# DTUWindEnergy/WindGym

Measured on AMD Instinct MI355X. Metric: env-steps/sec (whole node), 16-turbine farm x 4096 envs, higher is better.
Workload: dtype f32

## Files before the change

windgym_amd/csrc/wg_env.hip:

```cpp
#include <hip/hip_runtime.h>

#ifndef WG_ENV_ABLATE
#define WG_ENV_ABLATE 0
#endif
#include "wg_env_common.h"
#include "wg_internal.h"

struct __attribute__((aligned(16))) EnvSlotLds {
    int dev_rem, fill_rem, sub, budget;
    double s_new;
    int n_emit, n_valid, new_valid;
    unsigned n_emitted;
    float s_off_f, near_f, move_max, ti_pow;
    double s_off, ws;
    float ws_f, ti_f, wd_env, base_acc;
    int n_pushed, pend_farm_n, pend_base_n, n_flow;
    double c_time;
    int c_head;
    unsigned c_part, c_flow, c_istep, c_tag, n_emitted0;
    float out_pw;
    unsigned c_add;
    int bg_init;
    int pad_[3];
};
static_assert(sizeof(EnvSlotLds) == WG_ENV_SLOT_LDS_BYTES, "keep WG_ENV_SLOT_LDS_BYTES in sync (wg_flow.h)");
#define WG_ENV_OFF_SRC4 0
#define WG_ENV_OFF_REC4 1024
#define WG_ENV_OFF_RING 2048
#define WG_ENV_OFF_XR 3072
#define WG_ENV_OFF_SRC2 3584
#define WG_ENV_OFF_SL 4096
#define WG_ENV_OFF_HDR (WG_ENV_OFF_SL + 4 * WG_ENV_SLOT_LDS_BYTES)
#define WG_ENV_OFF_STAGE (WG_ENV_OFF_HDR + 128)
static_assert(WG_ENV_OFF_STAGE == WG_ENV_FIXED_LDS_BYTES, "keep WG_ENV_FIXED_LDS_BYTES in sync (wg_flow.h)");

__device__ __forceinline__ float env_slot_sums(const float v, const int N, const int NS, const int k, const int tid) {
    if (N == 16) return wg_row_sum(v);
    if (N < 16) {
        const int r = tid >> 4, i = tid & 15;
        const float x = __shfl(v, (r * N + i) & 63, 64);
        const float s = wg_row_sum((i < N && r < NS) ? x : 0.f);
        return __shfl(s, k << 4, 64);
    }
    const int h = tid >> 5, i = tid & 31;
    const float x = __shfl(v, (h * N + i) & 63, 64);
    float s = (i < N && h < NS) ? x : 0.f;
    WG_ROW_REDUCE(s, wg_addf)
    s += __shfl_xor(s, 16, 64);
    return __shfl(s, k << 5, 64);
}

static __device__ __forceinline__ void env_clone_dev(char* const smem, const int kd, const int N, const int P, const double dt_d,
                                                               float* const py_env, unsigned* const ra_env, const unsigned src,
                                                               const unsigned dst, const int lane) {
    float4* const Lsrc4 = reinterpret_cast<float4*>(smem + WG_ENV_OFF_SRC4);
    int4* const Lring = reinterpret_cast<int4*>(smem + WG_ENV_OFF_RING);
    float2* const Lsrc2 = reinterpret_cast<float2*>(smem + WG_ENV_OFF_SRC2);
    EnvSlotLds* const SL = reinterpret_cast<EnvSlotLds*>(smem + WG_ENV_OFF_SL);
    const int ga = (kd - 1) * N, gb = kd * N;
    const int4 last = Lring[ga + N - 1];
    const int nq = (last.x + last.y) >> 2;
    {
        const float4* const ps = reinterpret_cast<const float4*>(py_env + src);
        float4* const pd = reinterpret_cast<float4*>(py_env + dst);
        const uint4* const rs = reinterpret_cast<const uint4*>(ra_env + 2 * (size_t)src);
        uint4* const rd = reinterpret_cast<uint4*>(ra_env + 2 * (size_t)dst);
#pragma unroll 2
        for (int q = lane; q < nq; q += 64) {
            const float4 y = ps[q];
            const uint4 r0 = rs[q], r1 = rs[q + nq];
            pd[q] = y; rd[q] = r0; rd[q + nq] = r1;
        }
    }
    if (lane < N) {
        Lsrc4[gb + lane] = Lsrc4[ga + lane];
        Lsrc2[gb + lane] = Lsrc2[ga + lane];
        Lring[gb + lane].z = Lring[ga + lane].z;
    }
    if (lane == 0) {
        const EnvSlotLds& a = SL[kd - 1];
        EnvSlotLds& b = SL[kd];
        b.n_valid = a.n_valid; b.n_emitted = a.n_emitted; b.s_off = a.s_off;
        b.dev_rem = 0; b.sub = 0;
        b.budget = a.budget;
        double tm = a.c_time;
        for (int i = 0; i < a.n_flow; ++i) tm += dt_d;
        b.c_time = tm;
        int hd = a.c_head + (int)((a.n_emitted - a.n_emitted0) % (unsigned)P); if (hd >= P) hd -= P;
        b.c_head = hd; b.n_emitted0 = a.n_emitted;
        b.c_istep = a.c_istep + (unsigned)a.n_flow;
    }
}

template <bool NOISE, int WPE, int GLUE, int SPLIT>
__device__ __forceinline__ void env_flow(char* const smem, char* const smem_pass, float* const zone, const int wv, const int role, const int mode,
                                         const float* __restrict__ actions, const uint8_t* __restrict__ mask, const int chunk, EnvFlowOut& out) {
    const int tid = threadIdx.x & 63, e = blockIdx.x;
    int N, F, NS, NL;
    float inv_N;
    {
        const KArgsPtr ka = wg_cold_args();
        N = ka->p.N; F = ka->p.F; inv_N = ka->p.inv_N;
        NS = WPE == 2 ? F : 2 * F; NL = NS * N;
    }
    const int kbase = WPE == 2 ? wv * F : 0;
    const bool valid = tid < NL;
    const int g = valid ? tid : 0;
    const int k = (int)(((float)g + 0.5f) * inv_N);
    const int t = g - k * N;
    const int c = WPE == 2 ? wv : (F == 2 ? (k >> 1) : k), farm = F == 2 ? (k & 1) : 0;

    float4* const Lsrc4 = reinterpret_cast<float4*>(smem + WG_ENV_OFF_SRC4);
    uint4* const Lrec4 = reinterpret_cast<uint4*>(smem + WG_ENV_OFF_REC4);
    int4* const Lring = reinterpret_cast<int4*>(smem + WG_ENV_OFF_RING);
    double* const Lxr = reinterpret_cast<double*>(smem + WG_ENV_OFF_XR);
    float2* const Lsrc2 = reinterpret_cast<float2*>(smem + WG_ENV_OFF_SRC2);
    EnvSlotLds* const SL = reinterpret_cast<EnvSlotLds*>(smem + WG_ENV_OFF_SL);
    float* const def = reinterpret_cast<float*>(smem + WG_ENV_OFF_STAGE);
    float* const tiav = def + WG_ENV_CAP;
    unsigned short* const cl = reinterpret_cast<unsigned short*>(tiav + WG_ENV_CAP);
    unsigned short* const ql = reinterpret_cast<unsigned short*>(smem + WG_ENV_OFF_STAGE);
    EnvSlotLds& my = SL[k];

    WG_STAMP(0);
// ... 111 lines not shown
                const int dev0 = __shfl(dev_rem, WPE == 2 ? 0 : (env_live ^ 1) * F * N, 64);
                budget = wg_shadow_share(dev0 + gp.K * fill_max, total - env_steps_done, env_steps_done, e);
                budget = wg_shadow_share(dev_rem + gp.K * fill_rem, total - env_steps_done, env_steps_done, e, farm ? 0x80000000u : 0u);
                plan_left = total - env_steps_done;
            } else {
                const int inc = k0->p.env_inc;
                const long total = (long)((env_time_max_live + inc - 1) / inc) + 1;
                budget = role_dev ? wg_shadow_share(dev_rem + k0->p.K * fill_rem, total - env_steps_done, env_steps_done, e, farm ? 0x80000000u : 0u) : 0;
                plan_left = total - env_steps_done;
            }
        } else {
            role_dev = is_live_c && !masked_out;
            budget = chunk;
        }
        bool clone_here = false;
        if (k0->p.env_share) {
            const int dev_a = __shfl(dev_rem, (tid - N) & 63, 64);
            parked = valid && role_dev && farm == 1 && dev_rem > 0 && c_istep == 0u && dev_a > 0;
            const int twin_fill = __shfl(parked ? fill_rem + 1 : 0, (tid + N) & 63, 64);
            const bool lead = valid && role_dev && farm == 0 && twin_fill > 0;
            if (lead && mode == WG_MODE_STEP && !defer_init)
                budget = wg_shadow_share(dev_rem + k0->p.K * max(fill_rem, twin_fill - 1), plan_left, env_steps_done, e);
            if (parked) budget = 0;
            clone_here = lead && budget >= dev_rem;
        }
        if (SPLIT) {
            const bool two = valid && role_dev && budget >= 2;
            split_on = mode == WG_MODE_STEP && k0->p.K == 1 && (is_live_c || (SPLIT == 2 && !out.bg_init_pending)) && !defer_init && !__ballot(two) &&
                       !__ballot(clone_here);
            if (role == 1 && !split_on) return;
        }
        if (WPE == 2 && valid && t == 0) {
            my.dev_rem = dev_rem; my.fill_rem = fill_rem; my.bg_init = out.bg_init_pending; my.n_flow = 0; my.out_pw = 0.f;
        }
        {
            const bool any_work = valid && (role_live || (role_dev && budget > 0 && (dev_rem > 0 || fill_rem > 0)));
            if (!__ballot(any_work)) {
                if (WPE == 2 && mode == WG_MODE_STEP && !is_live_c && autoreset && role == 0) {
                    const int d0 = __shfl(dev_rem, 0, 64), f0 = __shfl(fill_rem, 0, 64), np0 = __shfl(n_pushed, 0, 64);
                    const KArgsPtr kf = wg_cold_args();
                    if (d0 == 0 && f0 == 0 && kf->d.gd->next_obs_ok != nullptr && kf->d.gd->next_obs_ok[ctx_id] == 0) {
                        out.first_obs = 1;
                        env_first_obs<GLUE != 0>((int)ctx_id, np0, tid);
                    }
                }
                return;
            }
        }

        const KArgsPtr k1 = wg_cold_args();
        const int rlen = l_rnext - l_roff;
        const int head = n_emitted == 0u ? rlen - 1 : fast_mod((int)(n_emitted - 1u), rlen, __builtin_amdgcn_rcpf((float)rlen));
        const float ws_f = (float)ws;
        if (valid) {
            Lxr[g] = l_xr;
            Lsrc4[g] = make_float4((float)l_xr, (float)l_yr, l_bnd.y, l_bnd.z);
            Lsrc2[g] = make_float2(l_bnd.x, l_bnd.w);
            Lring[g] = make_int4(l_roff, rlen, head, k);
            Lrec4[g] = make_uint4(0u, 0u, 0u, __float_as_uint(1.f));
            if (t == 0) {
                my.dev_rem = dev_rem; my.fill_rem = fill_rem; my.sub = 0; my.budget = budget;
                my.n_valid = n_valid; my.n_emitted = n_emitted; my.n_emitted0 = n_emitted;
                my.move_max = fabsf(k1->p.hill) * ws_f * k1->p.dt; my.ti_pow = fast_pow(ti_f, k1->p.tic);
                my.s_off = s_off; my.ws = ws; my.ws_f = ws_f; my.ti_f = ti_f; my.wd_env = wd_env; my.base_acc = 0.f;
                my.n_pushed = n_pushed; my.pend_farm_n = pend_farm_n; my.pend_base_n = pend_base_n; my.n_flow = 0;
                my.bg_init = out.bg_init_pending;
                my.c_time = c_time; my.c_head = c_head; my.c_part = c_part; my.c_flow = c_flow; my.c_istep = c_istep; my.c_tag = c_tag; my.c_add = c_add;
            }
        }
        float* const tabp = reinterpret_cast<float*>(smem + k1->p.env_off_tab);
        float* const tabct = tabp + n_tab;
        float2* const rpt = reinterpret_cast<float2*>(tabct + n_tab);
        const float hub = k1->p.hub;
        auto rp = [&](const float dy_, const float dz_) __attribute__((always_inline)) {
            const float dz = hub + dz_ - hub;
            return make_float2(dy_, dz * dz);
        };
        if (tid < n_tab) { tabp[tid] = pf_tp; tabct[tid] = pf_tc; }
        if (tid < S) rpt[tid] = rp(pf_dy, pf_dz);
        for (int i = tid + 64; i < n_tab; i += 64) { tabp[i] = k1->d.tab_power[i]; tabct[i] = k1->d.tab_ct[i]; }
        for (int i = tid + 64; i < S; i += 64) rpt[i] = rp(k1->d.rotor_dy[i], k1->d.rotor_dz[i]);

        yaw = l_yaw; tu = l_u; tti = l_ti; oyaw = l_yaw;
        if (role_live && farm == 0 && valid) {
            const float a = l_act, ymin = k1->p.yaw_min, ymax = k1->p.yaw_max, ystep = k1->p.yaw_step;
            if (k1->p.action_method == WG_ACT_YAW) {
                yaw = fminf(fmaxf(yaw + a * ystep, ymin), ymax);
            } else {
                float tf = a + 1.0f;
                tf = tf * 0.5f;
                tf = tf * (ymax - ymin);
                tf = tf + ymin;
                const float ny = fminf(fmaxf(tf, yaw - ystep), yaw + ystep);
                yaw = fminf(fmaxf(ny, ymin), ymax);
            }
        }
    }
    float tpow = 0.f, tct = 0.f, cg = 1.f;
    float sws = 0.f, swd = 0.f, syaw = 0.f, sp_ = 0.f;
    int part_acc = 0, stream_acc = 0;
    bool stepped = false;
    lds_barrier<64>();
    WG_STAMP(1);

    for (int round = 0;; ++round) {
        bool stepping, is_dev;
        int sub, K;
        if (__ballot(parked)) {
            bool due = parked && SL[k - 1].dev_rem == 0;
            unsigned long long due_m = __ballot(due);
            if (due_m) {
                full_barrier<64>();
                const KArgsPtr kc = wg_cold_args();
                const unsigned pstride = (unsigned)kc->p.pstride;
                const size_t pb_env = (size_t)(e * 2 * F + kbase) * pstride;
                const int src_lane = (tid - N) & 63;
                const float c_tu = __shfl(tu, src_lane, 64), c_tti = __shfl(tti, src_lane, 64), c_pw = __shfl(tpow, src_lane, 64);
                const float c_ct = __shfl(tct, src_lane, 64), c_cg = __shfl(cg, src_lane, 64);
                if (due) { tu = c_tu; tti = c_tti; tpow = c_pw; tct = c_ct; cg = c_cg; stepped = true; parked = false; }
                while (due_m) {
                    const int kd = __builtin_amdgcn_readlane(k, __builtin_ctzll(due_m));
                    env_clone_dev(smem, kd, N, kc->p.P, kc->p.dt_d, kc->d.py + pb_env, kc->d.rec_a + 2 * pb_env, (unsigned)(kd - 1) * pstride,
                                  (unsigned)kd * pstride, tid);
                    due_m &= ~(((1ull << N) - 1ull) << (kd * N));
                }
                lds_barrier<64>();
            }
        }
        {
            const KArgsPtr kr = wg_cold_args();
            K = kr->p.K;
            const int4 sch = *reinterpret_cast<const int4*>(&my.dev_rem);
            const bool active = sch.x > 0 || sch.y > 0;
            stepping = valid && (role_live ? (round < K) : (role_dev && active && (sch.w > 0 || sch.z != 0)));
            is_dev = !role_live && sch.x > 0;
            sub = sch.z;
            if (!__ballot(stepping)) break;
        out.rounds = round + 1;
            if (round > 0) full_barrier<64>();

            if (role_live && farm == 1 && stepping) {
                const float ystep = kr->p.yaw_step;
                if (kr->p.base_controller == WG_CTRL_LOCAL) {
                    const float off = 0.f - yaw;
                    const float sgn = (float)((off > 0.f) - (off < 0.f));
                    yaw = yaw + sgn * fminf(fabsf(off), ystep);
                } else {
                    const float sgn = (float)((yaw > 0.f) - (yaw < 0.f));
                    yaw = yaw - sgn * fminf(fabsf(yaw), ystep);
                }
            }

            if (stepping && t == 0) {
                const double dpart = kr->p.dpart;
                const int P = kr->p.P;
                const double s_off = my.s_off, adv = my.ws * kr->p.dt_d;
                double s_new = s_off + adv;
                int n_emit = 0;
                while (s_new >= dpart) { s_new -= dpart; ++n_emit; }
                if (n_emit > P) n_emit = P;
                int new_valid = my.n_valid + n_emit; if (new_valid > P) new_valid = P;
                my.s_new = s_new; my.n_emit = n_emit; my.new_valid = new_valid;
                my.s_off_f = (float)s_off;
                my.near_f = (float)(s_off + adv + dpart) + 0.01f;
            }
        }
        lds_barrier<64>();
        WG_STAMP(4);

        unsigned cmask = 0u;
        {
            const KArgsPtr kp = wg_cold_args();
            const float D = kp->p.D, inv_D = kp->p.inv_D, eps_max = kp->p.env_eps_max;
            const int gs0 = k * N;
            const float lim0 = kp->p.R_rot + 1.0e-3f * D;
            const float near_f = my.near_f, move_max = my.move_max;
            const float xt_f = Lsrc4[g].x, yt_f = Lsrc4[g].y;
#pragma unroll 4
            for (int s2 = 0; s2 < N; ++s2) {
                const float4 a = Lsrc4[gs0 + s2];
                const float2 b = Lsrc2[gs0 + s2];
                const float dxf = xt_f - a.x;
                const bool nearp = dxf < near_f;
                const float kb_ = nearp ? fmaxf(WG_K_MAX, a.z) : a.z, eb_ = nearp ? fmaxf(eps_max, a.w) : a.w;
                const float sig_max = (kb_ * (dxf * inv_D) + eb_) * D;
                const float bdv = b.x + (((__float_as_uint(b.y) != 0u) | nearp) ? move_max : 0.f);
                const float gap = fabsf(yt_f - a.y) - (5.0f * sig_max + bdv);
                const bool cd = (s2 != t) & (dxf >= 0.f) & (gap <= lim0);
                cmask |= cd ? (1u << s2) : 0u;
            }
            if (!stepping || (SPLIT && role == 1)) cmask = 0u;
        }
        int cbeg, nc;
        {
            const int cnt = __popc(cmask);
            const int inc = wg_wave_scan_i(cnt);
            cbeg = inc - cnt;
            nc = __builtin_amdgcn_readlane(inc, 63);
            unsigned m = cmask;
            int o = cbeg;
            while (m) { cl[o++] = (unsigned short)((g << 5) | __builtin_ctz(m)); m &= m - 1u; }
        }
        lds_barrier<64>();
        WG_STAMP(5);

        struct Cand { uint2 q0, q1; float y0, y1, xd, wgt; int en, jp0; bool ok, rest; };
        float dsum = 0.f, tia_max = 0.f;
        {
            const KArgsPtr kp = wg_cold_args();
            const unsigned pstride = (unsigned)kp->p.pstride;
            const size_t pb_env = (size_t)(e * 2 * F + kbase) * pstride;
            const uint2* const rc_env = reinterpret_cast<const uint2*>(kp->d.rec_a + 2 * pb_env);
            const float* const py_env = kp->d.py + pb_env;
            const double inv_dpart = kp->p.inv_dpart;
            const float inv_D = kp->p.inv_D;
            auto issue = [&](Cand& cd, const int cidx, const int c0, const int c1) __attribute__((always_inline)) {
                cd.ok = false; cd.rest = false;
// ... 155 lines not shown
            if (stepping) {
                const int4 rg = Lring[g];
                const unsigned mvl = __float_as_uint(Lsrc2[g].y);
                const int n_emit = my.n_emit;
                const bool full = (mvl != 0u && (int)(my.n_emitted - mvl) < rg.y) || n_emit >= 4 || n_emit >= rg.y;
                stream_acc += full ? rg.y : n_emit;
            }
        }
        if (stepping) {
            const float ti_f = my.ti_f;
            tu = my.ws_f;
            tu -= dsum;
            tti = __builtin_amdgcn_sqrtf(ti_f * ti_f + tia_max * tia_max);
        }
        lds_barrier<64>();
        WG_STAMP(9);

        if (!(SPLIT && split_on && role == 0)) {
            const KArgsPtr kp = wg_cold_args();
            const unsigned pstride = (unsigned)kp->p.pstride;
            const size_t pb_env = (size_t)(e * 2 * F + kbase) * pstride;
            float* const py_env = kp->d.py + pb_env;
            unsigned* const ra_env = kp->d.rec_a + 2 * pb_env;
            int nlist;
            {
                int cnt = 0, nqd = 0;
                bool full = false;
                if (stepping) {
                    const int4 rg = Lring[g];
                    const int rlen = rg.y, n_emit = my.n_emit;
                    const unsigned mvl = __float_as_uint(Lsrc2[g].y);
                    nqd = rlen >> 2;
                    const bool moving = mvl != 0u && (int)(my.n_emitted - mvl) < rlen;
                    full = moving || n_emit >= 4 || n_emit >= rlen;
                    stream_acc += full ? rlen : n_emit;
                    if (full) cnt = nqd;
                    else if (n_emit > 0) {
                        const unsigned sb = (unsigned)k * pstride + (unsigned)rg.x;
                        const uint4 rn = Lrec4[g];
                        const float y0 = Lsrc4[g].y;
#pragma unroll
                        for (int em = 0; em < 3; ++em) {
                            if (em < n_emit) {
                                int r = rg.z + 1 + em; if (r >= rlen) r -= rlen;
                                const unsigned ix = sb + (unsigned)r;
                                py_env[ix] = y0;
                                reinterpret_cast<uint2*>(ra_env)[ix] = make_uint2(rn.x, rn.y);
                            }
                        }
                    }
                }
                const int inc = wg_wave_scan_i(cnt);
                nlist = (WG_ENV_ABLATE & 2) ? 0 : __builtin_amdgcn_readlane(inc, 63);
                if (full) {
                    const int base = inc - cnt;
                    const unsigned tag = (unsigned)g << 10;
                    for (int i = 0; i < nqd; ++i) ql[base + i] = (unsigned short)(tag | (unsigned)i);
                }
            }
            lds_barrier<64>();
            WG_STAMP(10);
#ifdef WG_TIMELINE
            if (tid == 0) atomicAdd(&wg_counts[4], nlist);
#endif

            const float dpart_f = kp->p.dpart_f, inv_D = kp->p.inv_D, dt = kp->p.dt, eps0 = kp->p.eps0;
            struct QuadReq { float4 py; uint4 ra, rb; int g, kq; unsigned q; };
            auto request = [&](QuadReq& r, const int cidx) __attribute__((always_inline)) {
                const bool v = cidx < nlist;
                const unsigned en = v ? ql[cidx] : 0u;
                r.g = (int)(en >> 10); r.kq = (int)(en & 1023u);
                const int4 rg = Lring[r.g];
                r.q = (((unsigned)rg.w * pstride + (unsigned)rg.x) >> 2) + (unsigned)r.kq;
                if (v) {
                    r.py = reinterpret_cast<const float4*>(py_env)[r.q];
                    r.ra = reinterpret_cast<const uint4*>(ra_env)[2u * r.q];
                    r.rb = reinterpret_cast<const uint4*>(ra_env)[2u * r.q + 1u];
                }
            };
            auto advect_quad = [&](const QuadReq& cur, const int cidx) __attribute__((always_inline)) {
                if (cidx >= nlist) return;
                const int gq = cur.g, kq = cur.kq;
                const unsigned q = cur.q;
                const int4 rg = Lring[gq];
                const EnvSlotLds& sl = SL[rg.w];
                const int n_emit_q = sl.n_emit, n_valid_q = sl.n_valid;
                const float sof = sl.s_off_f;
                const int R = rg.y, hd = rg.z;
                const int r0 = 4 * kq;
                int j0 = hd - r0; if (j0 < 0) j0 += R;
                int e0 = r0 - hd - 1; if (e0 < 0) e0 += R;
                const bool emits = (e0 < n_emit_q) || (n_emit_q > 0 && e0 + 3 >= R);
                float pyv[4] = {cur.py.x, cur.py.y, cur.py.z, cur.py.w};
                unsigned rav[4] = {cur.ra.x, cur.ra.z, cur.rb.x, cur.rb.z};
                unsigned rbv[4] = {cur.ra.y, cur.ra.w, cur.rb.y, cur.rb.w};
#pragma unroll
                for (int i = 0; i < 4; ++i) {
                    int j = j0 - i; if (j < 0) j += R;
                    const float adv = m0_advect(pyv[i], rav[i], rbv[i], j, sof, dpart_f, inv_D, dt, eps0);
                    pyv[i] = j < n_valid_q ? adv : pyv[i];
                }
                const float y0 = Lsrc4[gq].y;
                if (emits) {
                    const uint4 rn = Lrec4[gq];
#pragma unroll
                    for (int i = 0; i < 4; ++i) {
                        int ei = e0 + i; if (ei >= R) ei -= R;
                        if (ei < n_emit_q) {
                            pyv[i] = y0; rav[i] = rn.x; rbv[i] = rn.y;
                        }
                    }
                    reinterpret_cast<uint4*>(ra_env)[2u * q] = make_uint4(rav[0], rbv[0], rav[1], rbv[1]);
                    reinterpret_cast<uint4*>(ra_env)[2u * q + 1u] = make_uint4(rav[2], rbv[2], rav[3], rbv[3]);
                }
                reinterpret_cast<float4*>(py_env)[q] = make_float4(pyv[0], pyv[1], pyv[2], pyv[3]);
                float ex = 0.f;
#pragma unroll
                for (int i = 0; i < 4; ++i) {
                    int j = j0 - i; if (j < 0) j += R;
                    if (j < n_valid_q) ex = fmaxf(ex, fabsf(pyv[i] - y0));
                }
                if (ex > Lsrc2[gq].x) atomicMax(reinterpret_cast<int*>(&Lsrc2[gq].x), __float_as_int(ex));
            };
            QuadReq qa, qb;
            qa.py = qb.py = make_float4(0.f, 0.f, 0.f, 0.f); qa.ra = qa.rb = qb.ra = qb.rb = make_uint4(0u, 0u, 0u, 0u);
            request(qa, tid);
            if (SPLIT && role == 1) {
                if (!env_flag_wait(reinterpret_cast<int*>(smem + WG_ENV_OFF_HDR))) atomicOr(kp->d.status, WG_STATUS_BIT_STATE);
            }
            for (int base = 0; base < nlist; base += 64) {
                qb = qa;
                request(qa, base + 64 + tid);
                advect_quad(qb, base + tid);
            }
        }
        lds_barrier<64>();
        WG_STAMP(3);
        if (SPLIT && role == 1) {
            if (stepping) reinterpret_cast<float4*>(wg_cold_args()->d.bnd)[(unsigned)((e * 2 * F + kbase) * N + g)].x = Lsrc2[g].x;
            return;
        }

        const bool measuring = stepping && !is_dev;
        const bool unit_end = measuring && (sub + 1 == K);
        const KArgsPtr kc = wg_cold_args();
        const float inv_k = 1.0f / (float)K;
        const unsigned ctx_id = (unsigned)(e * 2 + c);
        if (stepping) {
            {
                int4 rg = Lring[g];
                const int n_emit = my.n_emit;
                rg.z += n_emit;
                if (n_emit >= rg.y) rg.z %= rg.y; else if (rg.z >= rg.y) rg.z -= rg.y;
                Lring[g].z = rg.z;
                part_acc += min(my.new_valid, rg.y);
            }
            stepped = true;
            const int n_tab = kc->p.n_tab;
            const float tab_x0 = kc->p.tab_x0, tab_inv_dx = kc->p.tab_inv_dx;
            const float* const tabp = reinterpret_cast<const float*>(smem + kc->p.env_off_tab);
            const float wsn = fmaxf(tu * cg, 0.0f);
            tpow = env_tab(tabp, tab_x0, tab_inv_dx, n_tab, wsn);
            tct = env_tab(tabp + n_tab, tab_x0, tab_inv_dx, n_tab, wsn) * cg * cg;
            if (measuring && farm == 0) {
                const float wsm = __builtin_amdgcn_sqrtf(tu * tu);
                const float wdm = 0.f + my.wd_env;
                float val[WG_N_CH] = {sws + wsm, swd + wdm, syaw + yaw, sp_ + tpow};
                if (unit_end) {
// ... 101 lines not shown
            for (int i = 0; i < n_flow; ++i) tm += dt_d;
            const unsigned n_emitted = my.n_emitted;
            int hd = my.c_head + (int)((n_emitted - my.n_emitted0) % (unsigned)P); if (hd >= P) hd -= P;
            WgSlot& slot = ke->d.slot[(unsigned)(e * 2 * F + kbase + k)];
            slot.part_count = my.c_part + (unsigned)part_slot;
            slot.add_count = my.c_add + (unsigned)stream_slot;
            slot.head = hd; slot.n_valid = my.n_valid; slot.s_off = my.s_off; slot.time = tm;
            slot.istep = my.c_istep + (unsigned)n_flow; slot.n_emitted = n_emitted;
            slot.dev_remaining = my.dev_rem; slot.fill_remaining = my.fill_rem;
            slot.flow_count = my.c_flow + (unsigned)n_flow;
            WgCtx& cx = ke->d.ctx[(unsigned)(e * 2 + c)];
            if (farm == 0) { cx.n_pushed = my.n_pushed; cx.pend_farm_n = my.pend_farm_n; }
            if (farm == F - 1) cx.pend_base_n = my.pend_base_n;
        }
    }
    if (SPLIT) {
        out.g_yaw = yaw; out.g_old = oyaw; out.g_pw = tpow;
        out.g_pwb = F == 2 ? __shfl(tpow, min(tid + N, 63), 64) : 0.f;
    }
    WG_STAMP(8);
    if (mode == WG_MODE_STEP && (WPE == 1 || c != env_live) && !defer_init) {
        const EnvSlotLds& bs = SL[WPE == 2 ? 0 : (env_live ^ 1) * F];
        const int bctx = e * 2 + (env_live ^ 1);
        bool build = false;
        if (ke->p.autoreset && bs.dev_rem == 0 && bs.fill_rem == 0)
            build = bs.n_flow == 0 ? (ke->d.gd->next_obs_ok != nullptr && ke->d.gd->next_obs_ok[bctx] == 0) : out.truncates != 0;
        if (build) {
            const int np = bs.n_pushed;
            out.first_obs = 1;
            full_barrier<64>();
            env_first_obs<GLUE != 0>(bctx, np, tid);
        }
    }
    if (defer_init) {
        env_init_episode<GLUE != 0>(e, env_live ^ 1, tid);
        full_barrier<64>();
        if (valid && t == 0 && c != env_live) {
            const WgSlot& slot = ke->d.slot[(unsigned)(e * 2 * F + kbase + k)];
            my.dev_rem = slot.dev_remaining; my.fill_rem = slot.fill_remaining;
        }
        lds_barrier<64>();
    }
}


template <bool NOISE, int GLUE, int WPE, int SPLIT = 0>
__global__ void __launch_bounds__(64 * (WPE + SPLIT), WG_ENV_WAVES)
k_flow_env(const FlowP p_, const FlowPtrs d_, const int mode, const float* __restrict__ actions,
           const uint8_t* __restrict__ mask, const int chunk, const WgParams gp_, const WgPtrs gd_,
           float* __restrict__ obs_out, float* __restrict__ reward_out, uint8_t* __restrict__ trunc_out,
           float* __restrict__ final_obs_out) {
    extern __shared__ __attribute__((aligned(16))) char smem[];
#ifdef WG_TIMELINE
    if (threadIdx.x == 0) { for (int i = 0; i < 20; ++i) wg_stamps[i] = 0; wg_stamps[14] = wall_clock64(); for (int i = 0; i < 8; ++i) wg_counts[i] = 0; }
    __syncthreads();
#endif
    const int wv4 = WPE == 2 ? __builtin_amdgcn_readfirstlane((int)(threadIdx.x >> 6)) : 0;
    int wv = wv4, role = 0;
    if (SPLIT == 1 && wv4 == 2) {
        role = 1;
        wv = __builtin_amdgcn_readfirstlane(reinterpret_cast<const int*>(wg_cold_args()->d.env + blockIdx.x)[offsetof(WgEnv, live) / 4]) & 1;
    }
    if (SPLIT == 2) { wv = wv4 & 1; role = wv4 >> 1; }
    const int lds_wave = WPE == 2 ? wg_cold_args()->p.env_lds : 0;
    char* const sm = smem + wv4 * lds_wave;
    char* const sm_pass = smem + (SPLIT == 2 ? 2 + wv : 2) * lds_wave;
    float* const zone = SPLIT ? reinterpret_cast<float*>(smem + (2 + SPLIT) * lds_wave) : nullptr;
    EnvFlowOut fo;
    env_flow<NOISE, WPE, GLUE, SPLIT>(sm, sm_pass, zone, wv, role, mode, actions, mask, chunk, fo);
    if (SPLIT && role == 1) {
        if (GLUE != 0 && fo.truncates) { __builtin_amdgcn_s_waitcnt(0x0070); __syncthreads(); }
        return;
    }
    if (GLUE != 0) {
        full_barrier<64>();
        if (WPE == 2) {
            if (wv != fo.env_live) {
                const EnvKArgsPtr kb = (EnvKArgsPtr)wg_cold_args();
                const int e = (int)blockIdx.x;
                if (kb->p.autoreset && !fo.truncates && (threadIdx.x & 63) == 0) {
                    const int F = kb->p.F, K = kb->p.K;
                    const EnvSlotLds* const SLb = reinterpret_cast<const EnvSlotLds*>(sm + WG_ENV_OFF_SL);
                    int work = 0;
                    for (int f = 0; f < F; ++f) work = max(work, SLb[f].dev_rem + K * SLb[f].fill_rem);
                    env_bg_plan(kb, work, fo, e);
                }
                if (fo.bg_init_pending && (threadIdx.x & 63) == 0) kb->d.ctx[e * 2 + wv].init_pending = 0;
                if (fo.truncates) __builtin_amdgcn_s_waitcnt(0x0070);
            }
            if (fo.truncates) __syncthreads();
        }
        if (WPE == 1 || wv == fo.env_live) {
            const EnvKArgsPtr kg = (EnvKArgsPtr)wg_cold_args();
            const int F = kg->p.F, K = kg->p.K;
            const EnvSlotLds* const SLa = reinterpret_cast<const EnvSlotLds*>(sm + WG_ENV_OFF_SL);
            const int la = WPE == 2 ? 0 : fo.env_live * F, lb = (fo.env_live ^ 1) * F;
            const float fp = SLa[la].out_pw, bp = F == 2 ? SLa[la + 1].out_pw : 0.f;
            int work = 0;
            if (WPE == 1) for (int f = 0; f < F; ++f) work = max(work, SLa[lb + f].dev_rem + K * SLa[lb + f].fill_rem);
            const int hw = reinterpret_cast<const int*>(sm + WG_ENV_OFF_HDR)[threadIdx.x & 31];
            LeanFused fz;
            fz.pre = nullptr;
            if (SPLIT) {
                if (!env_flag_wait(reinterpret_cast<int*>(zone) + LEAN_PRE_FLAG)) atomicOr(kg->d.status, WG_STATUS_BIT_STATE);
                const int gl = (int)(threadIdx.x & 63), own = gl < kg->p.N ? gl : 0;
                fz.pre = zone;
#pragma unroll
                for (int ch = 0; ch < WG_N_CH; ++ch) fz.nw[ch] = __shfl(fo.g_nw[ch], own, 64);
                fz.yaw = fo.g_yaw; fz.old_yaw = fo.g_old; fz.pw = fo.g_pw; fz.pwb = fo.g_pwb;
            }
            WG_STAMP(12);
            env_glue<GLUE, WPE>(kg, fz, fp, bp, work, fo, hw);
            WG_STAMP(13);
        }
    }
#ifdef WG_TIMELINE
    {
        const KArgsPtr kt = wg_cold_args();
        if (threadIdx.x == 0 && kt->d.dbg) {
            wg_stamps[15] = wall_clock64();
            long long* row = kt->d.dbg + (size_t)blockIdx.x * 32;
            for (int kq = 0; kq < 16; ++kq) row[kq] = wg_stamps[kq];
            row[16] = fo.bg_init_pending; row[17] = fo.rounds; row[18] = fo.first_obs;
            row[19] = GLUE != 0 ? (long long)kt->d.env[blockIdx.x].timestep : 0;
            for (int kq = 0; kq < 8; ++kq) row[20 + kq] = wg_counts[kq];
            for (int kq = 0; kq < 4; ++kq) row[28 + kq] = wg_stamps[16 + kq];
        }
    }
#endif
}

template <bool NZ, int G>
static EnvKernel env_kernel(const int wpe, const int split) {
    if constexpr (G != 0) {
        if (split == 2) return k_flow_env<NZ, G, 2, 2>;
        if (split == 1) return k_flow_env<NZ, G, 2, 1>;
    }
    return wpe == 2 ? k_flow_env<NZ, G, 2> : k_flow_env<NZ, G, 1>;
}
static void env_launch(const FlowP* p, const FlowPtrs* d, const int glue, const int mode, const float* actions, const uint8_t* mask,
                       const int chunk, const WgParams* gp, const WgPtrs* gd, float* obs, float* reward, uint8_t* trunc,
                       float* final_obs, hipStream_t st) {
    const int wpe = p->env_wpe == 2 ? 2 : 1;
    const int split = glue != 0 && wpe == 2 && (p->env_split == 1 || p->env_split == 2) ? p->env_split : 0;
    const size_t lds = (size_t)p->env_lds * (wpe + split) + (split ? LEAN_PRE_BYTES : 0);
    const EnvKernel k = glue == 2 ? (p->noise ? env_kernel<true, 2>(wpe, split) : env_kernel<false, 2>(wpe, split))
                      : glue == 1 ? (p->noise ? env_kernel<true, 1>(wpe, split) : env_kernel<false, 1>(wpe, split))
                                  : (p->noise ? env_kernel<true, 0>(wpe, split) : env_kernel<false, 0>(wpe, split));
    hipLaunchKernelGGL(k, dim3(p->B), dim3(64 * (wpe + split)), lds, st, *p, *d, mode, actions, mask, chunk, *gp, *gd, obs, reward, trunc, final_obs);
}

extern "C" void wg_launch_flow_env(const FlowP* p, const FlowPtrs* d, int mode, const float* actions, const uint8_t* mask,
                                   int chunk, hipStream_t st) {
    static const WgParams gp0{};
    static const WgPtrs gd0{};
    env_launch(p, d, 0, mode, actions, mask, chunk, &gp0, &gd0, nullptr, nullptr, nullptr, nullptr, st);
}

extern "C" void wg_launch_step_env(const FlowP* p, const FlowPtrs* d, const WgParams* gp, const WgPtrs* gd, const float* actions,
                                   float* obs, float* reward, uint8_t* trunc, float* final_obs, hipStream_t st) {
    env_launch(p, d, gd->multi_out ? 2 : 1, WG_MODE_STEP, actions, nullptr, 0, gp, gd, obs, reward, trunc, final_obs, st);
}
```

windgym_amd/csrc/wg_plan.h:

```cpp
#pragma once
#include <algorithm>
#include <cmath>
#include <cstring>
#include <string>
#include <vector>

#ifndef __HIPCC__
struct float4;
#endif
#include "wg_flow.h"

struct WgHookInt {
    bool set = false;
    int v = 0;
};
struct WgHooks {
    WgHookInt flow_block, flow_res, flow_env, env_wpe, env_split, step_fused, sums, lds_pad, lf_cap, pstride_pad, step_graph, share_dev;
    bool first_obs_gl_only = false, no_box8 = false, debug = false, timeline = false;
    std::string timeline_out;
};

struct WgPlan {
    WgParams p;
    FlowP f;
// ... 293 lines not shown
    int env_cap, off_cl, off_tab;
    size_t bytes;
};
inline WgEnvbCarve wg_plan_envb_carve(const WgParams& p, int n_tab_u, int wpe) {
    WgEnvbCarve k;
    const int nlp = wpe == 4 ? 16 : 64;
    const int nl_w = (wpe == 4 ? 1 : (wpe == 2 ? p.F : 2 * p.F)) * p.N;
    k.env_cap = wpe == 4 ? 128 : 256;
    size_t ob = WG_ENVB_FIXED_LDS_BYTES(nlp) + (size_t)20 * k.env_cap;
    k.off_cl = (int)ob;
    ob = (ob + (size_t)2 * nl_w * (p.N > 1 ? p.N - 1 : 1) + 15) & ~(size_t)15;
    k.off_tab = (int)ob;
    ob += sizeof(float) * (2 * (size_t)n_tab_u + 2 * (size_t)p.S);
    k.bytes = (ob + 15) & ~(size_t)15;
    return k;
}

inline bool wg_plan_envb(const WgParams& p, const WgHooks& hk, FlowP& f, bool small, int lds_limit, int* wpe) {
    const int NL = 2 * p.F * p.N;
    *wpe = (p.B <= 2048) ? 2 : 1;
    if (hk.env_wpe.set) {
        const int w = hk.env_wpe.v;
        *wpe = (w == 4 && p.F == 2 && p.N <= 16) ? 4 : (w == 2 ? 2 : (w == 4 ? 2 : 1));
    }
    if (!(f.res && small && f.block == 64 && !f.gl && p.turb_mode >= WG_TURB_BOX && NL <= 64 && p.N <= 32 && p.P <= 4096 && f.S_pad <= 16 &&
          f.deficit_model == 0))
        return false;
    WgEnvbCarve k = wg_plan_envb_carve(p, f.n_tab, *wpe);
    while (*wpe > 1 && *wpe * k.bytes + 64 > (size_t)lds_limit) {
        *wpe /= 2;
        k = wg_plan_envb_carve(p, f.n_tab, *wpe);
    }
    f.env_cap = k.env_cap; f.envb_off_cl = k.off_cl; f.env_off_tab = k.off_tab; f.env_lds = (int)k.bytes;
    return f.env_lds <= 32768 && f.env_lds <= lds_limit;
}

inline void wg_plan_step_kernels(const wg_config* c, const WgHooks& hk, const WgParams& p, FlowP& f, bool small, int lds_limit) {
    const size_t qf = wg_plan_farm_quads(c, p);
    const bool env_ok = wg_plan_env(p, f, small, qf, lds_limit);
    int envb_wpe = 1;
    const bool envb_ok = wg_plan_envb(p, hk, f, small, lds_limit, &envb_wpe);
    f.env_inc = 1 + (p.extra_inc ? 1 : 0);
    f.env_eps_max = std::min(1.0f, (float)(p.eps0 * std::sqrt(3.0))) + 2.0f / 65535.0f;
    f.envw = ((env_ok || envb_ok) && !hk.flow_block.set && !hk.flow_res.set) ? 1 : 0;
    if (hk.flow_env.set) f.envw = ((env_ok || envb_ok) && hk.flow_env.v != 0) ? 1 : 0;
    f.env_wpe = (p.B <= 2048 && 2 * f.env_lds <= lds_limit) ? 2 : 1;
    if (hk.env_wpe.set) f.env_wpe = (hk.env_wpe.v == 2 && 2 * f.env_lds <= lds_limit) ? 2 : 1;
    const bool split_ok = env_ok && f.env_wpe == 2 && p.K == 1 && 4 * f.env_lds + 4096 <= lds_limit;
    f.env_split = (split_ok && p.B <= 1024 && qf >= 256) ? (p.B <= 512 ? 2 : 1) : 0;
    if (hk.env_split.set) f.env_split = (hk.env_split.v != 0 && split_ok && p.B <= 2048) ? (hk.env_split.v == 2 ? 2 : 1) : 0;
    if (envb_ok) f.env_wpe = envb_wpe;
    f.env_share = (f.envw && env_ok && p.F == 2) ? 1 : 0;
    if (hk.share_dev.set && hk.share_dev.v == 0) f.env_share = 0;
    const bool gen = p.turb_ti || p.farm_ti || p.farm_obs > 0 || (p.sum_mask_f | p.cur_mask_f) != 0;
    f.env_fused = (f.envw && p.sums_mode && !gen && p.power_avg <= 64) ? 1 : 0;
    if (hk.step_fused.set) f.env_fused = (f.env_fused && hk.step_fused.v != 0) ? 1 : 0;
}

inline void wg_plan_flow_scalars(const wg_config* c, const WgParams& p, double tab_x0, double tab_dx, FlowP& f) {
    f.B = p.B; f.N = p.N; f.F = p.F; f.K = p.K; f.P = p.P; f.S = p.S; f.NP = p.NP;
    f.S_pad = 1; f.S_shift = 0;
    while (f.S_pad < p.S) { f.S_pad <<= 1; f.S_shift++; }
    f.autoreset = p.autoreset; f.action_method = p.action_method; f.base_controller = p.base_controller;
    f.power_avg = p.power_avg; f.script_rows = 0; f.noise = (p.noise == WG_NOISE_NORMAL);
    f.dt = p.dt; f.D = p.D; f.inv_D = p.inv_D; f.hub = p.hub; f.dpart_f = (float)p.dpart; f.R_rot = 0.5f * p.D;
    f.inv_N = 1.0f / (float)p.N; f.inv_S = 1.0f / (float)p.S; f.inv_P = 1.0f / (float)p.P;
    f.inv_power_avg = 1.0f / (float)(p.power_avg > 0 ? p.power_avg : 1);
    f.pavg_magic = (unsigned)((1ull << 32) / (unsigned long long)(p.power_avg > 0 ? p.power_avg : 1)) + 1u;
    f.dt_d = p.dt_d; f.dpart = p.dpart; f.inv_dpart = 1.0 / p.dpart;
    f.yaw_min = p.yaw_min; f.yaw_max = p.yaw_max; f.yaw_step = p.yaw_step;
    f.ka = p.ka; f.kb = p.kb; f.eps0 = p.eps0; f.hill = p.hill; f.tia = p.tia; f.tib = p.tib; f.tic = p.tic; f.tid = p.tid;
    f.tab_x0 = (float)tab_x0; f.tab_inv_dx = (float)(1.0 / tab_dx);
    f.ue_scale = p.turb_mode == WG_TURB_NONE ? 1.0f : 2.0f;
    for (int i = 0; i < WG_N_CH; ++i) {
        f.hlen[i] = p.ring_cap[i]; f.ring_off[i] = p.ring_off[i]; f.fring_off[i] = p.fring_off[i];
        f.inv_hlen[i] = 1.0f / (float)p.ring_cap[i];
        f.hmagic[i] = (unsigned)((1ull << 32) / (unsigned long long)p.ring_cap[i]) + 1u;
        f.noise_sigma[i] = p.noise_sigma[i];
    }
    f.ring_stride = p.ring_stride; f.fring_stride = p.fring_stride;
    f.turb_mode = p.turb_mode; f.fc_scale = p.fc_scale; f.D_d = p.D_d; f.hub_d = p.hub_d;
    f.inv_sqrt_S = 1.0f / std::sqrt((float)p.S);
    f.added = (c->added_turbulence != 0 && c->turb_mode != WG_TURB_NONE) ? 1 : 0;
    f.no_ti_fold = c->no_ti_fold != 0; f.deficit_model = c->deficit_model;
    f.km1 = (float)wg_defd(c->m0_km1, 0.6); f.km2r = (float)(2.0 * wg_defd(c->m0_km2, 0.35) * 0.5 * p.D_d);
    f.sg_af = (float)wg_defd(c->m0_sg_af, 3.11); f.sg_bf = (float)wg_defd(c->m0_sg_bf, -0.68); f.sg_cf = (float)wg_defd(c->m0_sg_cf, 2.41);
    f.an_inv_ka = (float)(1.0 / wg_defd(c->m0_ka, 0.38));
}

inline int wg_plan_reset_launches(const wg_config* c, const WgParams& p, int reset_chunk) {
    double xmn = 1e300, xmx = -1e300, ymn = 1e300, ymx = -1e300;
    for (int t = 0; t < p.N; ++t) {
        xmn = std::min(xmn, c->x_pos[t]); xmx = std::max(xmx, c->x_pos[t]);
        ymn = std::min(ymn, c->y_pos[t]); ymx = std::max(ymx, c->y_pos[t]);
    }
    const double ext_x = xmx - xmn, ext_y = ymx - ymn;
    const double diag = std::sqrt(ext_x * ext_x + ext_y * ext_y);
    const double ws_lo = std::max(1e-3, std::min(c->ws_min, c->ws_max));
    const long max_dev = (long)std::ceil(2.0 * diag / ws_lo / c->dt_sim) + 2;
    const long max_work = max_dev + (long)p.K * (std::max(p.fill_a, p.fill_b) + 1);
    return (int)((max_work + reset_chunk - 1) / reset_chunk) + 1;
}

inline double wg_plan_alg_bytes(const WgParams& p) {
    const bool turb = p.turb_mode != WG_TURB_NONE, boxm = p.turb_mode >= WG_TURB_BOX;
    const double per_farm_step = (double)p.NP * (4 + 4 + 8 + (turb ? 24 : 0) + (boxm ? 64 : 0)) +
// ... 50 lines not shown
```

Baseline: 89.09 million.

## Write particle state to twin slot during step and clone only non-whole turbines

While the farm-0 env steps, its particle positions and records are also written to the parked twin slot's buffer. A per-turbine 'whole' mask records which turbines were fully rewritten this way. The later clone then copies only the remaining turbines' ranges, and skips the full barrier when none are left. This cuts global-memory copy traffic and a barrier on the clone path, at the cost of extra stores during stepping and global atomic counters for clone statistics on every clone.

```diff
diff --git a/windgym_amd/csrc/wg_env.hip b/windgym_amd/csrc/wg_env.hip
--- a/windgym_amd/csrc/wg_env.hip
+++ b/windgym_amd/csrc/wg_env.hip
@@ -1,4 +1,6 @@
 #include <hip/hip_runtime.h>
+
+#include <cassert>
 
 #ifndef WG_ENV_ABLATE
 #define WG_ENV_ABLATE 0
@@ -21,7 +23,7 @@
     float out_pw;
     unsigned c_add;
     int bg_init;
-    int pad_[3];
+    unsigned twin_q0, twin_q, whole;
 };
 static_assert(sizeof(EnvSlotLds) == WG_ENV_SLOT_LDS_BYTES, "keep WG_ENV_SLOT_LDS_BYTES in sync (wg_flow.h)");
 #define WG_ENV_OFF_SRC4 0
@@ -33,6 +35,10 @@
 #define WG_ENV_OFF_HDR (WG_ENV_OFF_SL + 4 * WG_ENV_SLOT_LDS_BYTES)
 #define WG_ENV_OFF_STAGE (WG_ENV_OFF_HDR + 128)
 static_assert(WG_ENV_OFF_STAGE == WG_ENV_FIXED_LDS_BYTES, "keep WG_ENV_FIXED_LDS_BYTES in sync (wg_flow.h)");
+__device__ unsigned wg_env_clone_stat[8];
+#ifdef WG_TIMELINE
+__shared__ int wg_cloned;
+#endif
 
 __device__ __forceinline__ float env_slot_sums(const float v, const int N, const int NS, const int k, const int tid) {
     if (N == 16) return wg_row_sum(v);
@@ -52,24 +58,30 @@
 
 static __device__ __forceinline__ void env_clone_dev(char* const smem, const int kd, const int N, const int P, const double dt_d,
                                                                float* const py_env, unsigned* const ra_env, const unsigned src,
-                                                               const unsigned dst, const int lane) {
+                                                               const unsigned dst, unsigned copy_m, const int lane) {
     float4* const Lsrc4 = reinterpret_cast<float4*>(smem + WG_ENV_OFF_SRC4);
     int4* const Lring = reinterpret_cast<int4*>(smem + WG_ENV_OFF_RING);
     float2* const Lsrc2 = reinterpret_cast<float2*>(smem + WG_ENV_OFF_SRC2);
     EnvSlotLds* const SL = reinterpret_cast<EnvSlotLds*>(smem + WG_ENV_OFF_SL);
     const int ga = (kd - 1) * N, gb = kd * N;
-    const int4 last = Lring[ga + N - 1];
-    const int nq = (last.x + last.y) >> 2;
-    {
-        const float4* const ps = reinterpret_cast<const float4*>(py_env + src);
-        float4* const pd = reinterpret_cast<float4*>(py_env + dst);
-        const uint4* const rs = reinterpret_cast<const uint4*>(ra_env + 2 * (size_t)src);
-        uint4* const rd = reinterpret_cast<uint4*>(ra_env + 2 * (size_t)dst);
-#pragma unroll 2
-        for (int q = lane; q < nq; q += 64) {
-            const float4 y = ps[q];
-            const uint4 r0 = rs[q], r1 = rs[q + nq];
-            pd[q] = y; rd[q] = r0; rd[q + nq] = r1;
+    if (copy_m != 0u && lane == 0) {
+        unsigned* const st = wg_env_clone_stat + (SL[kd - 1].twin_q0 != 0u ? 2 : 4);
+        atomicAdd(st, 1u); atomicAdd(st + 1, (unsigned)__popc(copy_m));
+    }
+    while (copy_m) {
+        const int tc = __builtin_ctz(copy_m);
+        copy_m &= copy_m - 1u;
+        const int4 rg = Lring[ga + tc];
+        const unsigned q0 = (unsigned)rg.x >> 2;
+        const int nq = rg.y >> 2;
+        const uint4* const ps = reinterpret_cast<const uint4*>(py_env + src) + q0;
+        uint4* const pd = reinterpret_cast<uint4*>(py_env + dst) + q0;
+        const uint4* const rs = reinterpret_cast<const uint4*>(ra_env + 2 * (size_t)src) + 2u * q0;
+        uint4* const rd = reinterpret_cast<uint4*>(ra_env + 2 * (size_t)dst) + 2u * q0;
+        for (int i = lane; i < 3 * nq; i += 64) {
+            const bool isp = i < nq;
+            const uint4 v = *(isp ? ps + i : rs + (i - nq));
+            *(isp ? pd + i : rd + (i - nq)) = v;
         }
     }
     if (lane < N) {
@@ -287,6 +299,7 @@
         const int rlen = l_rnext - l_roff;
         const int head = n_emitted == 0u ? rlen - 1 : fast_mod((int)(n_emitted - 1u), rlen, __builtin_amdgcn_rcpf((float)rlen));
         const float ws_f = (float)ws;
+        const bool twin_parked = __shfl((int)parked, (tid + N) & 63, 64) != 0;
         if (valid) {
             Lxr[g] = l_xr;
             Lsrc4[g] = make_float4((float)l_xr, (float)l_yr, l_bnd.y, l_bnd.z);
@@ -300,6 +313,8 @@
                 my.s_off = s_off; my.ws = ws; my.ws_f = ws_f; my.ti_f = ti_f; my.wd_env = wd_env; my.base_acc = 0.f;
                 my.n_pushed = n_pushed; my.pend_farm_n = pend_farm_n; my.pend_base_n = pend_base_n; my.n_flow = 0;
                 my.bg_init = out.bg_init_pending;
+                my.twin_q0 = (farm == 0 && k1->p.env_share == 1 && twin_parked) ? (unsigned)k1->p.pstride >> 2 : 0u;
+                my.twin_q = 0u; my.whole = 0u;
                 my.c_time = c_time; my.c_head = c_head; my.c_part = c_part; my.c_flow = c_flow; my.c_istep = c_istep; my.c_tag = c_tag; my.c_add = c_add;
             }
         }
@@ -345,7 +360,11 @@
             bool due = parked && SL[k - 1].dev_rem == 0;
             unsigned long long due_m = __ballot(due);
             if (due_m) {
-                full_barrier<64>();
+#ifdef WG_TIMELINE
+                if (tid == 0) wg_cloned = 1;
+#endif
+                const unsigned long long copy_all = __ballot(due && !((SL[k - 1].whole >> t) & 1u));
+                if (copy_all) full_barrier<64>();
                 const KArgsPtr kc = wg_cold_args();
                 const unsigned pstride = (unsigned)kc->p.pstride;
                 const size_t pb_env = (size_t)(e * 2 * F + kbase) * pstride;
@@ -356,7 +375,7 @@
                 while (due_m) {
                     const int kd = __builtin_amdgcn_readlane(k, __builtin_ctzll(due_m));
                     env_clone_dev(smem, kd, N, kc->p.P, kc->p.dt_d, kc->d.py + pb_env, kc->d.rec_a + 2 * pb_env, (unsigned)(kd - 1) * pstride,
-                                  (unsigned)kd * pstride, tid);
+                                  (unsigned)kd * pstride, (unsigned)((copy_all >> (kd * N)) & ((1ull << N) - 1ull)), tid);
                     due_m &= ~(((1ull << N) - 1ull) << (kd * N));
                 }
                 lds_barrier<64>();
@@ -398,6 +417,7 @@
                 my.s_new = s_new; my.n_emit = n_emit; my.new_valid = new_valid;
                 my.s_off_f = (float)s_off;
                 my.near_f = (float)(s_off + adv + dpart) + 0.01f;
+                my.twin_q = (is_dev && sch.x == 1) ? my.twin_q0 : 0u;
             }
         }
         lds_barrier<64>();
@@ -659,6 +679,17 @@
                 }
                 const int inc = wg_wave_scan_i(cnt);
                 nlist = (WG_ENV_ABLATE & 2) ? 0 : __builtin_amdgcn_readlane(inc, 63);
+                {
+                    const bool twinned = stepping && my.twin_q != 0u;
+                    if (__ballot(twinned)) {
+                        const unsigned long long fm = __ballot(full);
+                        if (twinned && t == 0) {
+                            const unsigned wm = (unsigned)((fm >> (k * N)) & ((1ull << N) - 1ull));
+                            my.whole = wm;
+                            atomicAdd(wg_env_clone_stat, 1u); atomicAdd(wg_env_clone_stat + 1, (unsigned)__popc(wm));
+                        }
+                    }
+                }
                 if (full) {
                     const int base = inc - cnt;
                     const unsigned tag = (unsigned)g << 10;
@@ -701,6 +732,7 @@
                 float pyv[4] = {cur.py.x, cur.py.y, cur.py.z, cur.py.w};
                 unsigned rav[4] = {cur.ra.x, cur.ra.z, cur.rb.x, cur.rb.z};
                 unsigned rbv[4] = {cur.ra.y, cur.ra.w, cur.rb.y, cur.rb.w};
+                const bool twinned = __ballot(sl.twin_q != 0u) != 0ull && sl.twin_q != 0u;
 #pragma unroll
                 for (int i = 0; i < 4; ++i) {
                     int j = j0 - i; if (j < 0) j += R;
@@ -708,7 +740,7 @@
                     pyv[i] = j < n_valid_q ? adv : pyv[i];
                 }
                 const float y0 = Lsrc4[gq].y;
-                if (emits) {
+                if (emits || twinned) {
                     const uint4 rn = Lrec4[gq];
 #pragma unroll
                     for (int i = 0; i < 4; ++i) {
@@ -719,8 +751,14 @@
                     }
                     reinterpret_cast<uint4*>(ra_env)[2u * q] = make_uint4(rav[0], rbv[0], rav[1], rbv[1]);
                     reinterpret_cast<uint4*>(ra_env)[2u * q + 1u] = make_uint4(rav[2], rbv[2], rav[3], rbv[3]);
+                    if (twinned) {
+                        uint4* const tw = reinterpret_cast<uint4*>(ra_env + 2 * (size_t)pstride) + 2u * q;
+                        tw[0] = make_uint4(rav[0], rbv[0], rav[1], rbv[1]);
+                        tw[1] = make_uint4(rav[2], rbv[2], rav[3], rbv[3]);
+                    }
                 }
                 reinterpret_cast<float4*>(py_env)[q] = make_float4(pyv[0], pyv[1], pyv[2], pyv[3]);
+                if (twinned) reinterpret_cast<float4*>(py_env + pstride)[q] = make_float4(pyv[0], pyv[1], pyv[2], pyv[3]);
                 float ex = 0.f;
 #pragma unroll
                 for (int i = 0; i < 4; ++i) {
@@ -928,7 +966,7 @@
            float* __restrict__ final_obs_out) {
     extern __shared__ __attribute__((aligned(16))) char smem[];
 #ifdef WG_TIMELINE
-    if (threadIdx.x == 0) { for (int i = 0; i < 20; ++i) wg_stamps[i] = 0; wg_stamps[14] = wall_clock64(); for (int i = 0; i < 8; ++i) wg_counts[i] = 0; }
+    if (threadIdx.x == 0) { for (int i = 0; i < 20; ++i) wg_stamps[i] = 0; wg_stamps[14] = wall_clock64(); for (int i = 0; i < 8; ++i) wg_counts[i] = 0; wg_cloned = 0; }
     __syncthreads();
 #endif
     const int wv4 = WPE == 2 ? __builtin_amdgcn_readfirstlane((int)(threadIdx.x >> 6)) : 0;
@@ -997,7 +1035,7 @@
             wg_stamps[15] = wall_clock64();
             long long* row = kt->d.dbg + (size_t)blockIdx.x * 32;
             for (int kq = 0; kq < 16; ++kq) row[kq] = wg_stamps[kq];
-            row[16] = fo.bg_init_pending; row[17] = fo.rounds; row[18] = fo.first_obs;
+            row[16] = fo.bg_init_pending; row[17] = fo.rounds | (wg_cloned << 8); row[18] = fo.first_obs;
             row[19] = GLUE != 0 ? (long long)kt->d.env[blockIdx.x].timestep : 0;
             for (int kq = 0; kq < 8; ++kq) row[20 + kq] = wg_counts[kq];
             for (int kq = 0; kq < 4; ++kq) row[28 + kq] = wg_stamps[16 + kq];
@@ -1017,6 +1055,7 @@
 static void env_launch(const FlowP* p, const FlowPtrs* d, const int glue, const int mode, const float* actions, const uint8_t* mask,
                        const int chunk, const WgParams* gp, const WgPtrs* gd, float* obs, float* reward, uint8_t* trunc,
                        float* final_obs, hipStream_t st) {
+    assert(p->env_share == 0 || p->pstride % 4 == 0);
     const int wpe = p->env_wpe == 2 ? 2 : 1;
     const int split = glue != 0 && wpe == 2 && (p->env_split == 1 || p->env_split == 2) ? p->env_split : 0;
     const size_t lds = (size_t)p->env_lds * (wpe + split) + (split ? LEAN_PRE_BYTES : 0);
@@ -1026,6 +1065,14 @@
     hipLaunchKernelGGL(k, dim3(p->B), dim3(64 * (wpe + split)), lds, st, *p, *d, mode, actions, mask, chunk, *gp, *gd, obs, reward, trunc, final_obs);
 }
 
+extern "C" int wg_env_clone_stats(unsigned* out, int reset) {
+    unsigned z[8] = {0, 0, 0, 0, 0, 0, 0, 0};
+    if (hipDeviceSynchronize() != hipSuccess) return -1;
+    if (out && hipMemcpyFromSymbol(out, HIP_SYMBOL(wg_env_clone_stat), sizeof(z)) != hipSuccess) return -1;
+    if (reset && hipMemcpyToSymbol(HIP_SYMBOL(wg_env_clone_stat), z, sizeof(z)) != hipSuccess) return -1;
+    return 0;
+}
+
 extern "C" void wg_launch_flow_env(const FlowP* p, const FlowPtrs* d, int mode, const float* actions, const uint8_t* mask,
                                    int chunk, hipStream_t st) {
     static const WgParams gp0{};
diff --git a/windgym_amd/csrc/wg_plan.h b/windgym_amd/csrc/wg_plan.h
--- a/windgym_amd/csrc/wg_plan.h
+++ b/windgym_amd/csrc/wg_plan.h
@@ -369,6 +369,7 @@
     if (envb_ok) f.env_wpe = envb_wpe;
     f.env_share = (f.envw && env_ok && p.F == 2) ? 1 : 0;
     if (hk.share_dev.set && hk.share_dev.v == 0) f.env_share = 0;
+    if (hk.share_dev.set && hk.share_dev.v == 2 && f.env_share) f.env_share = 2;
     const bool gen = p.turb_ti || p.farm_ti || p.farm_obs > 0 || (p.sum_mask_f | p.cur_mask_f) != 0;
     f.env_fused = (f.envw && p.sums_mode && !gen && p.power_avg <= 64) ? 1 : 0;
     if (hk.step_fused.set) f.env_fused = (f.env_fused && hk.step_fused.v != 0) ? 1 : 0;
```

Result: slower. 88.20 million (-1.0%).
